# aniketntnu/WordDiffusion

Measured on AMD Instinct MI355X. Metric: denoised 64x256 word images/sec (1000-step DDPM), whole job, higher is better.
Workload: dtype bf16x3; 1 GPU; BASELINE configs[1]: batch 64 per GPU of 64x256 crops = [64,4,8,32] latents, 1000-step DDPM (999 executed steps), base unet.py UNetModel (320 ch, mult (1,1), 4 heads, 339 writers), random-init synthetic weights; variant=base, batch_per_gpu=64, noise_steps=1000, executed_steps_per_image=999, precision=split-bf16 MFMA x3, fp32 accumulate (<=1e-4 of the fp32 reference), output_finite=True

## Files before the change

worddiffusion_amd/csrc/wd_gemm.hip:

```cpp
#include <stdlib.h>

#include "wd_common.h"
#include "wd_gemm_epi.h"
#include "wd_gemm_priv.h"


namespace {

constexpr int BK = 32;

__device__ __forceinline__ int lds_off(int row, int ch) { return row * 64 + ((ch ^ ((row >> 2) & 3)) << 4); }
__device__ __forceinline__ int lds_off16(int row, int ch) { return row * 64 + ((ch ^ ((0 - (row >> 2)) & 3)) << 4); }


template <int BM, int BN, int TN, int NT>
__device__ __forceinline__ void wd_epilogue_lds(const wd_gemm_args& a, const f32x16 (&acc)[TN], char* smem, const int m0,
                                                const int n0, const int wm, const int wn, const int wcols, const int kh,
                                                const int nkh, const int tid, const int sidx = 0) {
    constexpr int LDE = BN + 4;
    float* ep = reinterpret_cast<float*>(smem);
    const int lane = tid & 63;
    const int frow = lane & 31, fhalf = lane >> 5;
    asm volatile("s_waitcnt vmcnt(0)" ::: "memory");
    __syncthreads();
// ... 2113 lines not shown
    if (a.rowvec && a.rowvec_ld <= 0) return WD_EINVAL;
    if (a.resid && a.resid_ld <= 0) return WD_EINVAL;
    {
        const int nout = a.act == WD_ACT_GEGLU ? a.n / 2 : a.n;
        if ((a.out_f32 && a.out_ld < nout) || (a.out_hi && a.out_pl_ld < nout) || (a.resid && a.resid_ld < nout) ||
            (a.rowvec && a.rowvec_ld < nout))
            return WD_EINVAL;
        for (int s = 0; s < a.nsrc; ++s)
            if (!(s == 0 && a.a32) && a.src[s].ld < a.src[s].c) return WD_EINVAL;
    }

    if (a.w_layout == 3) {
        bool ok = a.src[0].ntaps <= 9 && (a.nsrc == 1 || (a.src[1].gather == nullptr && a.src[1].ntaps == 1));
        for (int s = 0; s < a.nsrc; ++s) ok = ok && (a.src[s].c % 64 == 0);
        if (!ok) return WD_EINVAL;
        const wd_src& q0 = a.src[0];
        const bool same3 = q0.ntaps == 9 && q0.gather && a.slab_rows > 0 && q0.hw_src == a.hw_out && a.hw_out % a.slab_rows == 0;
        const bool down3 = a.tile == 64080 && q0.ntaps == 9 && q0.gather && a.slab_rows > 0 && q0.hw_src == 4 * a.hw_out;
        if (!same3 && !down3) a.slab_rows = 0;
        a.tickets = nullptr;
        if (a.tile == 64080) {
            if (!wd_gemmq_applies(a)) return WD_EINVAL;
            if (a.gn_gamma && (40 % a.gn_cpg || 80 % a.gn_cpg)) return WD_EINVAL;
            r.a = a, r.kernel = K_GEMMQ;
            return WD_OK;
        }
        const int nk64 = a.ktot / 64;
        if (a.ksplit == 0) a.ksplit = a.ws ? wd_auto_ksplit(a.tile, a.m, a.n, nk64, a.ws_floats) : 1;
        if (a.ksplit > 1 && (nk64 < a.ksplit || (long)a.ksplit * a.m * a.n > a.ws_floats)) a.ksplit = 1;
        if (a.gn_gamma && a.ksplit <= 1) return WD_EINVAL;
        {
            static const bool slab_env = getenv("WDIFF_GEMMW_SLAB") ? atoi(getenv("WDIFF_GEMMW_SLAB")) != 0 : WD_GEMMW_SLAB_DEFAULT;
            const bool want = (a.dbg & WD_GEMMW_SLAB_OFF) ? false : (a.dbg & WD_GEMMW_SLAB_ON) ? true : slab_env;
            const bool fits = a.tile == 64320 && a.npass == 3 && a.ksplit <= 1 && a.w_ngroups <= 1 && !a.a32 && !a.ln_gamma && same3 &&
                              64 % a.slab_rows == 0 && a.hw_out % 64 == 0 && a.m % a.hw_out == 0 && q0.c % 64 == 0 &&
                              (a.nsrc == 1 || (a.src[1].gather == nullptr && a.src[1].ntaps == 1));
            a.dbg &= ~(WD_GEMMW_SLAB_OFF | WD_GEMMW_SLAB_ON);
            if (want && fits) a.dbg |= WD_GEMMW_SLAB_BIT;
        }
        r.a = a, r.kernel = K_GEMMW;
        return WD_OK;
    }
#ifndef WDIFF_EXPERIMENTAL
    if (a.w_layout == 1) return WD_EINVAL;
#else
    if (a.w_layout == 1) {
        if (a.src[0].ntaps > 9 || a.slab_rows <= 0) return WD_EINVAL;
        if (a.nsrc == 2 && (a.src[1].gather || a.src[1].ntaps != 1)) return WD_EINVAL;
        if (a.tile == 0) a.tile = (a.act == WD_ACT_GEGLU || a.n % 160) ? 128064 : 128160;
        if (a.act == WD_ACT_GEGLU && a.n % (a.tile % 1000)) return WD_EINVAL;
        if (a.slab_rows > 192) return WD_EINVAL;
        if (a.tile != 128064 && a.tile != 128128 && a.tile != 128160) return WD_EINVAL;
        r.a = a, r.kernel = K_SLAB;
        return WD_OK;
    }
#endif
    bool conv3 = false;
    if (a.w_layout == 2) {
        const wd_src& q0 = a.src[0];
        static const int conv3_mode = getenv("WDIFF_CONV3") ? atoi(getenv("WDIFF_CONV3")) : 0;
#ifdef WDIFF_EXPERIMENTAL
        const bool conv3_env = conv3_mode != 0 || (a.dbg & 0x1000);
#else
        const bool conv3_env = false;
        (void)conv3_mode;
#endif
        const bool same3 = q0.ntaps == 9 && q0.gather && a.slab_rows > 0 && q0.hw_src == a.hw_out && a.hw_out % a.slab_rows == 0;
        conv3 = conv3_env && same3 && q0.c % 64 == 0 && a.act != WD_ACT_GEGLU && (a.tile == 0 || a.tile == 128160) &&
                (a.nsrc == 1 || (!a.src[1].gather && a.src[1].ntaps == 1 && a.src[1].c % 64 == 0));
        if (conv3) a.tile = 128160;
// ... 150 lines not shown
```

worddiffusion_amd/csrc/wd_gemm_priv.h:

```cpp
#pragma once
#include "wd_common.h"

int wd_gemmw_launch(const wd_gemm_args& a, hipStream_t st);
constexpr bool WD_GEMMW_SLAB_DEFAULT = true;
constexpr int WD_GEMMW_SLAB_OFF = 0x8000, WD_GEMMW_SLAB_ON = 0x10000, WD_GEMMW_SLAB_BIT = WD_GEMMW_SLAB_ON;
int wd_gemm_launch_reduce(const wd_gemm_args& a, hipStream_t st, int bm);
bool wd_gemmq_applies(const wd_gemm_args& a);
int wd_gemmq_launch(const wd_gemm_args& a, hipStream_t st);
```

worddiffusion_amd/csrc/wd_gemmw.hip:

```cpp
#include "wd_gemm_epi.h"
#include "wd_gemm_priv.h"

namespace {

constexpr int WNT = 512;

typedef __attribute__((ext_vector_type(4))) unsigned w_u32x4;

__device__ __forceinline__ int w_lds_off(int row, int ch) { return row * 128 + ((ch ^ ((row >> 1) & 7)) << 4); }

template <int NPASS, int RH, bool A32, bool SLAB = false>
__global__ void __launch_bounds__(WNT, 1) wd_gemmw_kernel(const wd_gemm_args a, const int nbn, const int nbm) {
#if defined(__HIP_DEVICE_COMPILE__)
    static_assert(!SLAB || (NPASS == 3 && RH == 1 && !A32), "the slab form is the split-bf16 64 x 320 kernel over operand planes");
    constexpr int NPL = (NPASS == 1) ? 1 : 2;
    constexpr int BM = 64 * RH, BN = 320 / RH;
    constexpr int A_PL = BM * 128;
    constexpr int STAGE = NPL * A_PL;
    constexpr uint32_t WD_OOB = 0x80000000u;

    extern __shared__ __attribute__((aligned(16))) char smem[];
    const int Wm = SLAB ? a.slab_rows : 1, wsh = __builtin_ctz(Wm);
    const int TR = 64 >> wsh, NR = TR + 2, SW = Wm + 2;
    const int CPL = NR * SW * 128, CHB = 2 * CPL;
    int* s_tab = reinterpret_cast<int*>(smem + 2 * STAGE);

    const int ntile = nbn * nbm;
    const int nwg = ntile * a.ksplit;
    int wg;
    {
        const int bid = blockIdx.x;
        const int q = nwg >> 3, r = nwg & 7, xcd = bid & 7, loc = bid >> 3;
        wg = (xcd < r ? xcd * (q + 1) : r * (q + 1) + (xcd - r) * q) + loc;
    }
    const int sidx = wg % a.ksplit;
    wg /= a.ksplit;
    const int bn_i = wg % nbn, bm_i = wg / nbn;
    const int m0 = bm_i * BM, n0 = bn_i * BN;

    const int tid = threadIdx.x;
    const int lane = tid & 63;
    const int wave = __builtin_amdgcn_readfirstlane(tid >> 6);
    const int kh = wave >> 2;
    const int rh = RH == 2 ? (wave >> 1) & 1 : 0;
    const int cg = RH == 2 ? wave & 1 : wave & 3;
    const int l15 = lane & 15, lq = lane >> 4;

    if constexpr (!SLAB) {
        const int nt0 = a.src[0].ntaps;
        const int32_t* g0 = a.src[0].gather;
        const int hw_src0 = a.src[0].hw_src;
        const int Wimg = a.slab_rows;
        for (int idx = tid; idx < nt0 * BM; idx += WNT) {
            const int t = idx / BM, row = idx - t * BM;
            const int m = m0 + row;
            int v = -1;
            if (m < a.m) {
                if (g0 && Wimg > 0) {
                    const int b = m / a.hw_out, p = m - b * a.hw_out;
                    const int y = p / Wimg, x = p - y * Wimg;
                    const int ky = t / 3, dy = ky - 1, dx = t - ky * 3 - 1;
                    const int sy = y + dy, sx = x + dx;
                    if (sy >= 0 && sy * Wimg < a.hw_out && sx >= 0 && sx < Wimg) v = b * hw_src0 + sy * Wimg + sx;
                } else if (g0) {
                    const int b = m / a.hw_out, p = m - b * a.hw_out;
                    const int g = g0[t * a.hw_out + p];
                    if (g >= 0) v = b * hw_src0 + g;
                } else {
                    v = m;
                }
            }
            s_tab[idx] = v;
        }
    }
    float* s_aff = reinterpret_cast<float*>(s_tab + 9 * BM);
    if constexpr (A32) {
        const int c0 = a.src[0].c;
        const int b = m0 / a.hw_out;
        const int ngp = c0 / a.a32_pcpg, ratio = a.a32_cpg / a.a32_pcpg;
        for (int c = tid; c < c0; c += WNT) {
            const int g = c / a.a32_cpg;
            double su = 0.0, sq = 0.0;
            for (int k = 0; k < ratio; ++k)
                for (int ck = 0; ck < a.a32_nchunk; ++ck) {
                    const double* pp = a.a32_part + (((long)b * a.a32_nchunk + ck) * ngp + g * ratio + k) * 2;
                    su += pp[0];
                    sq += pp[1];
                }
            const double n = (double)a.src[0].hw_src * a.a32_cpg;
            const double mu = su / n;
            double var = sq / n - mu * mu;
            if (var < 0.0) var = 0.0;
            const float rstd = (float)(1.0 / sqrt(var + (double)a.a32_eps));
            const float sc = rstd * a.a32_gamma[c];
            s_aff[2 * c] = sc;
            s_aff[2 * c + 1] = a.a32_beta[c] - (float)mu * sc;
        }
    }
    __syncthreads();
    unsigned long long skipmask = 0;
    if (!SLAB && RH == 1 && a.src[0].gather) {
        for (int t = 0; t < a.src[0].ntaps; ++t) {
            const unsigned long long oob = __ballot(s_tab[t * BM + lane] < 0);
#pragma unroll
            for (int i = 0; i < 4; ++i)
                if (((oob >> (16 * i)) & 0xFFFFull) == 0xFFFFull) skipmask |= 1ull << (4 * t + i);
        }
    }

    auto make_srd = [](const wd_bf16* p) {
        return __builtin_amdgcn_make_buffer_rsrc(const_cast<wd_bf16*>(p), 0, 0x7FFFFFF0, 0x00020000);
    };
    const int nct = a.n >> 4;
    const long wgrp = a.w_ngroups > 1 ? (long)((m0 % a.hw_out) / (a.hw_out / a.w_ngroups)) * a.w_group_stride : 0;
    const __amdgpu_buffer_rsrc_t srd_w_hi = make_srd(a.w_hi + wgrp), srd_w_lo = make_srd((a.w_lo ? a.w_lo : a.w_hi) + wgrp);
    const uint32_t b_voff = (uint32_t)(((n0 >> 4) + 5 * cg) * 1024 + lane * 16);
    const uint32_t kstep_bytes = (uint32_t)nct * 1024u;

    const int arow = tid >> 3, ach = tid & 7;
    const int a_dst = w_lds_off(arow, ach);

    const int nk_all = a.ktot / 64;
    const int cpt0 = a.src[0].c >> 6, n0st = a.src[0].ntaps * cpt0;
    const int k_begin = __builtin_amdgcn_readfirstlane((int)((long)nk_all * sidx / a.ksplit));
    const int k_end = __builtin_amdgcn_readfirstlane((int)((long)nk_all * (sidx + 1) / a.ksplit));
    const int nk = SLAB ? 0 : k_end - k_begin;
    int s = 0, tap = 0, kc = 0, left;
    int cur_ld = a.src[0].ld, cur_cpt = cpt0;
    if (k_begin < n0st) {
        tap = __builtin_amdgcn_readfirstlane(k_begin / cpt0);
        kc = k_begin - tap * cpt0;
// ... 153 lines not shown
                        acc[i][t] = __builtin_amdgcn_mfma_f32_16x16x32_bf16(xa[i][0], fb[t][NPL - 1], acc[i][t], 0, 0, 0);
                    }
                    acc[i][t] = __builtin_amdgcn_mfma_f32_16x16x32_bf16(xa[i][0], fb[t][0], acc[i][t], 0, 0, 0);
                }
            }
        }
    };
    const uint32_t cpt0_inv = (65536u + (uint32_t)cpt0 - 1u) / (uint32_t)cpt0;
    auto skip_of = [&](const int kit) {
        if constexpr (RH != 1) return 0;
        const int ka = k_begin + kit;
        const int tp = (int)(((uint32_t)ka * cpt0_inv) >> 16);
        int sk = (ka < n0st && ka < 1024) ? (int)((skipmask >> (4 * tp)) & 15ull) : 0;
        if (kit >= nk) sk = 15;
        return __builtin_amdgcn_readfirstlane(sk);
    };

    if constexpr (SLAB) {
        const wd_src& q0 = a.src[0];
        const int H = a.hw_out >> wsh;
        const int bsm = m0 / a.hw_out;
        const int y0 = (m0 - bsm * a.hw_out) >> wsh;
        const int ntok = NR * Wm;
        const int cpt1 = a.nsrc > 1 ? a.src[1].c >> 6 : 0, nch = cpt0 + cpt1;
        const int nst = 9 * cpt0 + cpt1;
        int skm0 = 0, skm2 = 0;
        int ub[4];
#pragma unroll
        for (int i = 0; i < 4; ++i) {
            if (y0 + ((16 * i + 15) >> wsh) < 1) skm0 |= 1 << i;
            if (y0 + ((16 * i) >> wsh) + 1 >= H) skm2 |= 1 << i;
            ub[i] = ((16 * i) >> wsh) * SW + ((16 * i) & (Wm - 1));
        }
        const uint32_t frow_bytes = (uint32_t)(q0.ld * 2), frow1_bytes = (uint32_t)(a.src[1].ld * 2);
        int fdst = -1;
        auto slab_piece = [&](const int t, const int chunk, const bool live) -> uint32_t {
            int ln;
            asm volatile("v_mbcnt_lo_u32_b32 %0, -1, 0\n\tv_mbcnt_hi_u32_b32 %0, -1, %0" : "=v"(ln));
            const int tq = wave * 8 + (ln >> 3) + 64 * t, fpc = ln & 7;
            if (chunk >= cpt0) {
                const bool piece = live && tq < 64;
                fdst = piece ? w_lds_off(tq, fpc) : -1;
                return piece ? (uint32_t)(m0 + tq) * frow1_bytes + (uint32_t)(fpc * 16) : WD_OOB;
            }
            const int fy = tq >> wsh, fx = tq & (Wm - 1);
            const int gy = y0 - 1 + fy;
            const bool piece = live && tq < ntok;
            fdst = piece ? w_lds_off(fy * SW + fx + 1, fpc) : -1;
            return (piece && gy >= 0 && gy < H) ? (uint32_t)(bsm * q0.hw_src + gy * Wm + fx) * frow_bytes + (uint32_t)(fpc * 16) : WD_OOB;
        };
        auto slab_load = [&](const int t, const int chunk, const bool live) {
            const uint32_t vo = slab_piece(t, chunk, live);
            if (chunk < cpt0) {
                ra[0][0] = __builtin_amdgcn_raw_buffer_load_b128(srd0_hi, vo, chunk * 128, 0);
                ra[0][1] = __builtin_amdgcn_raw_buffer_load_b128(srd0_lo, vo, chunk * 128, 0);
            } else {
                ra[0][0] = __builtin_amdgcn_raw_buffer_load_b128(srd1_hi, vo, (chunk - cpt0) * 128, 0);
                ra[0][1] = __builtin_amdgcn_raw_buffer_load_b128(srd1_lo, vo, (chunk - cpt0) * 128, 0);
            }
        };
        auto slab_store = [&](char* buf, const int t, const int chunk, const bool live) {
            slab_piece(t, chunk, live);
            if (fdst >= 0) {
                *reinterpret_cast<w_u32x4*>(buf + fdst) = ra[0][0];
                *reinterpret_cast<w_u32x4*>(buf + CPL + fdst) = ra[0][1];
            }
        };
        for (int i = tid; i < 2 * 2 * NR * 2 * 8; i += WNT) {
            const int pc = i & 7, side = (i >> 3) & 1;
            int rest = i >> 4;
            const int ry = rest % NR;
            rest /= NR;
            const int pl = rest & 1, bf = rest >> 1;
            *reinterpret_cast<w_u32x4*>(smem + bf * CHB + pl * CPL + w_lds_off(ry * SW + (side ? SW - 1 : 0), pc)) = w_u32x4{0u, 0u, 0u, 0u};
        }
        kb = 0;
        load_b(xb, true);
        {
            w_u32x4 v[3][2];
#pragma unroll
            for (int t = 0; t < 3; ++t) {
                slab_load(t, 0, true);
                v[t][0] = ra[0][0], v[t][1] = ra[0][1];
            }
#pragma unroll
            for (int t = 0; t < 3; ++t) {
                ra[0][0] = v[t][0], ra[0][1] = v[t][1];
                slab_store(smem, t, 0, true);
            }
        }
        int st = 0, sc = 0;
        int pft = 0, pfc = -1;
        auto mem_phase = [&](const int kit, bf16x8 (&bnext)[5][NPL]) {
            const bool conv = sc < cpt0;
            if (pfc >= 0) slab_store(smem + (pfc & 1) * CHB, pft, pfc, true);
            int tn = st + 1, cn = sc;
            if (tn == (conv ? 9 : 1)) tn = 0, cn = sc + 1;
            kb = cn < cpt0 ? tn * cpt0 + cn : n0st + cn - cpt0;
            load_b(bnext, kit + 1 < nst);
            const bool two = !conv || (st == 8 && sc == cpt0 - 1);
            const int fc = two ? sc + 2 : sc + 1, ft = two ? 0 : st;
            const bool freal = fc < nch && 64 * ft < (fc < cpt0 ? ntok : 64);
            pfc = freal ? fc : -1, pft = ft;
            if (freal) slab_load(ft, fc, true);
            const int ky = (st * 11) >> 5;
            const int shift = ky * SW + (st - 3 * ky);
            const char* cb = smem + (sc & 1) * CHB;
            int ln;
            asm volatile("v_mbcnt_lo_u32_b32 %0, -1, 0\n\tv_mbcnt_hi_u32_b32 %0, -1, %0" : "=v"(ln));
            const int f15 = ln & 15, ch = kh * 4 + (ln >> 4);
            const int frow = conv ? shift + (f15 >> wsh) * SW + (f15 & (Wm - 1)) : f15;
#pragma unroll
            for (int i = 0; i < 4; ++i) {
                const int ao = w_lds_off((conv ? ub[i] : 16 * i) + frow, ch);
#pragma unroll
                for (int p = 0; p < NPL; ++p) xa[i][p] = *reinterpret_cast<const bf16x8*>(cb + p * CPL + ao);
// ... 137 lines not shown
    const int nct = n >> 4;
    const int l = (int)(i & 63);
    const long blk = i >> 6;
    const int ct = (int)(blk % nct);
    const long ks = blk / nct;
    const long src = (long)(ct * 16 + (l & 15)) * ktot + ks * 32 + (l >> 4) * 8;
    reinterpret_cast<uint4*>(out_hi)[i] = *reinterpret_cast<const uint4*>(hi + src);
    if (lo) reinterpret_cast<uint4*>(out_lo)[i] = *reinterpret_cast<const uint4*>(lo + src);
}

template <int NPASS, int RH, bool A32 = false>
int launchw(const wd_gemm_args& a, hipStream_t st) {
    constexpr int NPL = (NPASS == 1) ? 1 : 2;
    constexpr int BM = 64 * RH, BN = 320 / RH;
    constexpr int loop_smem = 2 * NPL * BM * 128 + 9 * BM * 4 + (A32 ? 2 * 1024 * 4 : 0);
    constexpr int red_smem = BM * (BN + 4) * 4 + WD_STAT_SCRATCH;
    constexpr int smem = loop_smem > red_smem ? loop_smem : red_smem;
    static bool attr_done = false;
    if (!attr_done) {
        if (hipFuncSetAttribute(reinterpret_cast<const void*>(&wd_gemmw_kernel<NPASS, RH, A32>), hipFuncAttributeMaxDynamicSharedMemorySize,
                                smem) != hipSuccess)
            return WD_ELAUNCH;
        attr_done = true;
    }
    const int nbn = a.n / BN, nbm = (a.m + BM - 1) / BM;
    {
        WdLaunchScope scope(WD_CLS_GEMM_WDIRECT, st, 2.0 * (double)a.m * (double)a.n * (double)a.ktot);
        hipLaunchKernelGGL((wd_gemmw_kernel<NPASS, RH, A32>), dim3(nbn * nbm * a.ksplit), dim3(WNT), smem, st, a, nbn, nbm);
    }
    if (a.ksplit > 1) return wd_gemm_launch_reduce(a, st, BM);
    return wd_check_launch();
}

int launchw_slab(const wd_gemm_args& a, hipStream_t st) {
    constexpr int red_smem = 64 * (320 + 4) * 4 + WD_STAT_SCRATCH;
    constexpr int max_loop = 2 * 2 * 198 * 128;
    constexpr int max_smem = max_loop > red_smem ? max_loop : red_smem;
    static_assert(max_smem <= 160 * 1024, "LDS budget");
    const int W = a.slab_rows;
    const int loop_smem = 2 * 2 * (64 / W + 2) * (W + 2) * 128;
    const int smem = loop_smem > red_smem ? loop_smem : red_smem;
    static bool attr_done = false;
    if (!attr_done) {
        if (hipFuncSetAttribute(reinterpret_cast<const void*>(&wd_gemmw_kernel<3, 1, false, true>), hipFuncAttributeMaxDynamicSharedMemorySize,
                                max_smem) != hipSuccess)
            return WD_ELAUNCH;
        attr_done = true;
    }
    const int nbn = a.n / 320, nbm = a.m / 64;
    {
        WdLaunchScope scope(WD_CLS_GEMM_WDIRECT, st, 2.0 * (double)a.m * (double)a.n * (double)a.ktot);
        hipLaunchKernelGGL((wd_gemmw_kernel<3, 1, false, true>), dim3(nbn * nbm), dim3(WNT), smem, st, a, nbn, nbm);
    }
    return wd_check_launch();
}

}

int wd_gemmw_launch(const wd_gemm_args& a, hipStream_t st) {
    if (a.dbg & WD_GEMMW_SLAB_BIT) return launchw_slab(a, st);
    if (a.a32) return launchw<3, 1, true>(a, st);
    if (a.tile == 128160) return a.npass == 3 ? launchw<3, 2>(a, st) : launchw<1, 2>(a, st);
    return a.npass == 3 ? launchw<3, 1>(a, st) : launchw<1, 1>(a, st);
}

extern "C" int wd_gemm_pack_w(const wd_bf16* hi, const wd_bf16* lo, int n, int ktot, wd_bf16* out_hi, wd_bf16* out_lo, void* stream) {
    if (!hi || !out_hi || (lo && !out_lo) || n <= 0 || ktot <= 0 || n % 16 || ktot % 32) return WD_EINVAL;
    const long total = (long)n * ktot / 8;
    hipStream_t st = reinterpret_cast<hipStream_t>(stream);
    WdLaunchScope scope(WD_CLS_OTHER, st);
    hipLaunchKernelGGL(wd_pack_w_kernel, dim3((unsigned)((total + 255) / 256)), dim3(256), 0, st, hi, lo, n, ktot, out_hi, out_lo);
    return wd_check_launch();
}
```

worddiffusion_amd/engine.py:

```python
from __future__ import annotations

import collections
import ctypes as C
import math
import os
from typing import Dict, List, Optional, Tuple

import numpy as np
import torch

from . import _native as N
from .layers import (DownsampleParams, ResBlockParams, SpatialTransformerParams, UpsampleParams)


def conv_gather_table(h: int, w: int, mode: str) -> Tuple[np.ndarray, int, int]:
    if mode == "same":
        ho, wo = h, w
    elif mode == "down":
        ho, wo = (h + 2 - 3) // 2 + 1, (w + 2 - 3) // 2 + 1
    elif mode == "up":
        ho, wo = 2 * h, 2 * w
    elif mode == "down_rb":
        ho, wo = (h - 2) // 2 + 1, (w - 2) // 2 + 1
    else:
# ... 76 lines not shown
def slab_span(tab: Optional[np.ndarray], hw_out: int, hw_src: int, m: int, bm: int = 128) -> int:
    if tab is None:
        return bm
    period = int(np.lcm(bm, hw_out))
    mt = min(m, 2 * period)
    rows = np.arange(mt)
    b, p = rows // hw_out, rows % hw_out
    src = np.where(tab[:, p] >= 0, b[None, :] * hw_src + tab[:, p], -1)
    span = 0
    for r0 in range(0, mt, bm):
        blk = src[:, r0:r0 + bm]
        valid = blk[blk >= 0]
        if valid.size:
            span = max(span, int(valid.max() - valid.min() + 1))
    return span


_PARAM_GEN = [0]
_NATIVE_WRITES = [0]


def note_native_write():
    _NATIVE_WRITES[0] += 1

PLAN_CACHE_SIZE = int(os.environ.get("WDIFF_PLAN_CACHE", "4"))


def _bump_param_gen(*_a):
    _PARAM_GEN[0] += 1


torch.nn.modules.module.register_module_parameter_registration_hook(_bump_param_gen)

FILM_CHUNK_ROWS = int(os.environ.get("WDIFF_FILM_CHUNK_ROWS", "8192"))


class _Recipe:
    __slots__ = ("name", "planes", "rows", "cols", "shape", "pieces")

    def __init__(self, name, planes, rows=0, cols=0, shape=None):
        self.name, self.planes, self.rows, self.cols, self.shape, self.pieces = name, planes, rows, cols, shape, []

    @staticmethod
    def _nct(w):
        return w.shape[0], w.shape[1], (w.shape[2] * w.shape[3] if w.dim() == 4 else 1)

    def fwd(self, w, row_off=0, col_off=0, g=0):
        n, c, t = self._nct(w)
        assert row_off + n <= self.rows and col_off + t * c <= self.cols, self.name
        self.pieces.append((0, w, None, n, c, t, row_off, col_off, 0, g))
        return self

    def bwd(self, w, col_off=0, npad=None):
        n, c, t = self._nct(w)
        npad = n if npad is None else npad
        assert c <= self.rows and col_off + t * npad <= self.cols, self.name
        self.pieces.append((1, w, None, n, c, t, 0, col_off, npad, 0))
        return self

    def vec(self, p, p2=None, off=0, g=0):
        self.pieces.append((2, p, p2, p.numel(), 1, 1, 0, off, 0, g))
        return self

    def host(self) -> torch.Tensor:
        first = self.pieces[0][1]
        out = torch.zeros((self.rows, self.cols) if self.planes else (int(torch.tensor(self.shape).prod()),),
# ... 128 lines not shown
        raise ValueError(f"writer_keep must be a bool / uint8 tensor [{B}], False or None, got {k.dtype} {tuple(k.shape)}")
    return (k != 0).to(torch.uint8)


def _ptr(t: Optional[torch.Tensor], byte_off: int = 0):
    return None if t is None else t.data_ptr() + byte_off


class UNetEngine:

    fold_proj = False

    def __init__(self, model, variant: str):
        self.model = model
        self.variant = variant
        self.lib = N.lib()
        self.npass = 3
        self._sig = None
        self._ps, self._ps_gen = None, -1
        self._pack = None
        self._w: Dict[str, torch.Tensor] = {}
        self._w3: Dict[str, torch.Tensor] = {}
        self._w3_meta: Dict[str, tuple] = {}
        self._wf: Dict[str, torch.Tensor] = {}
        self.use_wdirect = os.environ.get("WDIFF_GEMM_WDIRECT", "1") != "0"
        self.gemmw_slab = {None: None, "0": False}.get(os.environ.get("WDIFF_GEMMW_SLAB"), True)
        self.use_up_phases = os.environ.get("WDIFF_UPSAMPLE_PHASES", "1") != "0"
        self._derived: Dict[str, tuple] = {}
        self.use_smallmap = os.environ.get("WDIFF_GEMM_SMALLMAP", "1") != "0"
        self.fuse_ff = os.environ.get("WDIFF_FUSE_FF", "1") != "0"
        self.fuse_proj = os.environ.get("WDIFF_FUSE_PROJ", "1") != "0"
        self.fuse_ln = os.environ.get("WDIFF_FUSE_LN", "1") != "0"
        self.fuse_gn_in = int(os.environ.get("WDIFF_FUSE_GN_IN", "1"))
        self.use_slab = os.environ.get("WDIFF_SLAB", "0") != "0"
        self.fuse_stats = os.environ.get("WDIFF_FUSE_STATS", "1") != "0"
        self.fuse_xattn = os.environ.get("WDIFF_FUSE_XATTN", "1") != "0"
        self.use_conv3 = os.environ.get("WDIFF_CONV3", "0") != "0"
        if (self.use_slab or self.use_conv3) and not self.lib.wd_gemm_experimental():
            raise N.NativeError("WDIFF_SLAB / WDIFF_CONV3 need a library built with WDIFF_EXPERIMENTAL=1 "
                                "(python -m worddiffusion_amd.build --force)")
        self.fuse_xattn_pair = os.environ.get("WDIFF_FUSE_XATTN_PAIR", "1") != "0"
        self.fuse_st = os.environ.get("WDIFF_FUSE_ST", "1") != "0"
        self.fold_proj = os.environ.get("WDIFF_FOLD_PROJ", "1") != "0"
        self.fuse_out = os.environ.get("WDIFF_FUSE_OUT", "1") != "0"
        self.fuse_in = os.environ.get("WDIFF_FUSE_IN", "1") != "0"
        self.pack_kv = os.environ.get("WDIFF_PACK_KV", "1") != "0"
        self.fuse_gn2 = os.environ.get("WDIFF_FUSE_GN2", "1") != "0"
        self.fuse_gn = os.environ.get("WDIFF_FUSE_GN", "1") != "0"
        self.fuse_split = os.environ.get("WDIFF_FUSE_SPLIT", "1") != "0"
        self._plans: Dict[tuple, Plan] = {}
        self._tabs: Dict[tuple, torch.Tensor] = {}
        self._tab_np: Dict[int, np.ndarray] = {}
        self._same_w: Dict[int, int] = {}
        self._down_w: Dict[int, int] = {}
        self._ws = None
        self.device = None

    def set_precision(self, mode: str):
        npass = {"bf16x3": 3, "fp32": 3, "bf16": 1}[mode]
        if npass != self.npass:
            self.npass = npass
            self._plans.clear()

    def _recipes(self) -> "RecipeBook":
        m = self.model
        R = RecipeBook()
# ... 246 lines not shown
        s.lo = planes[1].data_ptr() + 2 * col_off
        s.gather = _ptr(gather)
        s.ld, s.c, s.ntaps, s.hw_src = ld, c, ntaps, hw_src
        return s

    def _gemm(self, ops, what, srcs, wname, m, hw_out, bias=None, rowvec=None, rowvec_ld=0, resid=None,
              resid_ld=0, resid_rows=None, act=N.ACT_NONE, out_f32=None, out_ld=0, out_pl=None, n=None, tile=0,
              w_row_off=0, want_stats=False, a32=None, ln=None, w_groups=None):
        a = N.WdGemmArgs()
        for i, s in enumerate(srcs):
            a.src[i] = s
        a.nsrc = len(srcs)
        a.npass = self.npass
        wp = self._w[wname]
        ktot = wp.shape[2]
        assert ktot == sum(s.ntaps * s.c for s in srcs), (what, ktot, [(s.ntaps, s.c) for s in srcs])
        nrows = wp.shape[1] if n is None else n
        a.w_hi = wp[0].data_ptr() + 2 * w_row_off * ktot
        a.w_lo = wp[1].data_ptr() + 2 * w_row_off * ktot
        a.m, a.n, a.ktot, a.hw_out = m, nrows, ktot, hw_out
        a.bias = _ptr(bias)
        a.rowvec, a.rowvec_ld = rowvec, rowvec_ld
        a.resid, a.resid_ld, a.resid_rows = resid, resid_ld, resid_rows
        a.act = act
        a.out_f32, a.out_ld = _ptr(out_f32), out_ld
        if out_pl is not None:
            a.out_hi, a.out_lo, a.out_pl_ld = out_pl[0].data_ptr(), out_pl[1].data_ptr(), out_pl.shape[2]
        if a32 is not None:
            self._set_a32(a, *a32)
        if w_groups is not None:
            a.w_ngroups, a.w_group_stride = w_groups
        a.tile = tile
        if self._ws is None:
            self._ws = torch.empty(128 * 128 * 160 * 8, dtype=torch.float32, device=self.device)
        a.ksplit, a.ws, a.ws_floats = 0, self._ws.data_ptr(), self._ws.numel()
        self._give_tickets(a, m, nrows)
        span = 0
        if self.use_slab and w_row_off == 0 and (len(srcs) == 1 or (srcs[1].ntaps == 1 and not srcs[1].gather)):
            tabnp = getattr(srcs[0], "_tab_np", None)
            span = slab_span(tabnp, hw_out, srcs[0].hw_src, m)
            if span > 192 or ((m + 127) // 128) * max(1, nrows // 160) < 96:
                span = 0
        s0 = srcs[0]
        frag = not span and not self.use_conv3 and w_row_off == 0 and n is None and act == N.ACT_NONE and tile == 0
        width = (getattr(s0, "_down_w", 0) or getattr(s0, "_same_w", 0)) if s0.ntaps == 9 else 0
        wdirect = (frag and self.use_wdirect and wdirect_fills_chip(m, nrows) and
                   self._legal(a, w_layout=3, tile=64320, slab_rows=getattr(s0, "_same_w", 0) if s0.ntaps == 9 else 0))
        smallmap = (frag and not wdirect and self.use_smallmap and hw_out == 64 and 128 <= (m // 64) * (nrows // 80) <= 512 and
                    self._legal(a, w_layout=3, tile=64080, slab_rows=width))
        assert (a32 is None and w_groups is None) or wdirect, what
        if wdirect or smallmap:
            wf = self._wfrag(wname)
            a.w_hi, a.w_lo = wf[0].data_ptr(), wf[1].data_ptr()
            if wdirect and self.gemmw_slab is not None:
                a.dbg |= 0x10000 if self.gemmw_slab else 0x8000
        elif span:
            meta = (srcs[0].ntaps, srcs[0].c, srcs[1].c if len(srcs) > 1 else 0)
            if wname not in self._w3:
                self._w3[wname] = slab_order(wp, *meta)
                self._w3_meta[wname] = meta
            assert self._w3_meta[wname] == meta, wname
            w3 = self._w3[wname]
            a.w_hi, a.w_lo = w3[0].data_ptr(), w3[1].data_ptr()
            a.w_layout, a.slab_rows = 1, span
        else:
            same_w = getattr(srcs[0], "_same_w", 0)
            if (same_w and srcs[0].ntaps == 9 and srcs[0].c % 64 == 0 and act == N.ACT_NONE and tile == 0 and
                    (len(srcs) == 1 or (srcs[1].ntaps == 1 and not srcs[1].gather and srcs[1].c % 64 == 0))):
                a.w_layout, a.slab_rows = 2, same_w
        a._ln_pl = None
        if ln is not None and self.fuse_ln and not self.use_slab:
            pl = torch.zeros((2, m, nrows), dtype=torch.bfloat16, device=self.device)
            if self._legal(a, out_hi=pl[0].data_ptr(), out_lo=pl[1].data_ptr(), out_pl_ld=nrows, ln_gamma=self._w[ln + ".g"].data_ptr(),
                           ln_beta=self._w[ln + ".b"].data_ptr(), ln_eps=1e-5):
                self._cur_plan.keep.append(pl)
                a._ln_pl = pl
        stats = None
        if want_stats and self.fuse_stats and nrows % 32 == 0 and (hw_out % 128 == 0 or hw_out == 64) and not span:
            cpg = nrows // 32
            r = self._resolved(a, stat_part=a.ws, stat_cpg=cpg)
            if r is not None:
                nchunk = max(1, hw_out // (r.tile // 1000))
                part = torch.zeros((m // hw_out, nchunk, 32, 2), dtype=torch.float64, device=self.device)
                self._cur_plan.keep.append(part)
                a.stat_part, a.stat_cpg = part.data_ptr(), cpg
                stats = (part, nchunk, cpg)
        a._stats = stats
        self._cur_plan.keep.append(a)
        ops.append((self.lib.wd_gemm, (C.byref(a),), what))
        return a

    def _resolved(self, a, **fields) -> Optional[N.WdGemmArgs]:
        b = N.WdGemmArgs.from_buffer_copy(a)
        for k, v in fields.items():
            setattr(b, k, v)
        out = N.WdGemmArgs()
        return out if self.lib.wd_gemm_check(C.byref(b), C.byref(out)) == N.WD_OK else None

    def _legal(self, a, apply=True, **fields) -> bool:
        if self._resolved(a, **fields) is None:
            return False
        if apply:
            for k, v in fields.items():
                setattr(a, k, v)
        return True

    def _set_a32(self, a, x32: "Act", gname, eps, silu):
        part, nchunk, pc = x32.stats
        a.a32, a.a32_ld, a.a32_part = x32.t.data_ptr(), x32.c, part.data_ptr()
        a.a32_nchunk, a.a32_pcpg, a.a32_cpg = nchunk, pc, x32.c // 32
        a.a32_gamma, a.a32_beta = self._w[gname + ".g"].data_ptr(), self._w[gname + ".b"].data_ptr()
        a.a32_eps, a.a32_silu = float(eps), int(silu)

    def _wdirect_ok(self, srcs, m, n, hw_out, a32=None, **fields) -> bool:
        a = N.WdGemmArgs()
        for i, s in enumerate(srcs):
            a.src[i] = s
        a.nsrc, a.npass, a.m, a.n, a.ktot, a.hw_out = len(srcs), self.npass, m, n, sum(s.ntaps * s.c for s in srcs), hw_out
        a.w_layout, a.tile = 3, 64320
        a.w_hi = a.w_lo = a.out_f32 = 16
        a.out_ld = n
        if a32 is not None:
            self._set_a32(a, *a32)
        return self._legal(a, apply=False, **fields)

    def _give_tickets(self, a, m, n):
        ntick = ((m + 63) // 64) * ((n + 63) // 64)
        if ntick > 2048:
            return
        P = self._cur_plan
        tk = getattr(P, "_tickets", None)
        if tk is None or P._ticket_off + ntick > tk.numel():
            tk = torch.zeros(1 << 16, dtype=torch.int32, device=self.device)
            P.keep.append(tk)
            P._tickets, P._ticket_off = tk, 0
        a.tickets, a.ntickets = tk.data_ptr() + 4 * P._ticket_off, ntick
        P._ticket_off += ntick

    def _gn(self, P, ops, what, srcs: List[Act], gname, eps, silu, want_raw=False, dropout=None):
        B = self._B
        h, w = srcs[0].h, srcs[0].w
        hw = h * w
        ctot = sum(s.c for s in srcs)
        cpg = ctot // 32
        has_perm = any(s.perm is not None for s in srcs)
        if has_perm and not (len(srcs) == 2 and srcs[1].perm is None and self.fuse_gn2 and not any(s.c % cpg for s in srcs)):
            raise NotImplementedError(f"{what}: a phase-major map (Upsample) is read by the two-source GroupNorm of a decoder block only")
        if any(s.c % cpg for s in srcs):
            cat = self._f32(P, B * hw, ctot)
            coff = 0
            for s in srcs:
                ops.append((self.lib.wd_copy2d, (cat.data_ptr() + 4 * coff, 4 * ctot, s.t.data_ptr(), 4 * s.c, 4 * s.c,
                                                 B * hw), what + ":concat"))
                coff += s.c
            srcs = [Act(cat, ctot, h, w)]
        pl = self._planes(P, B * hw, ctot)
        raw = self._planes(P, B * hw, ctot) if want_raw else None
# ... 19 lines not shown
        rhi, rlo = self._hilo(raw)
        if len(todo) == 2 and self.fuse_gn2:
            (sa, pa, na, pca, ca), (sb, pb, nb_, pcb, cb) = todo
            ops.append((self.lib.wd_gn_apply2,
                        (sa.t.data_ptr(), sa.c, sa.c, pa.data_ptr(), na, pca, ca, sb.t.data_ptr(), sb.c, sb.c, pb.data_ptr(), nb_, pcb, cb,
                         B, hw, cpg, gam.data_ptr(), bet.data_ptr(), eps, int(silu), hi, lo, ctot, rhi, rlo,
                         sa.perm.data_ptr() if sa.perm is not None else None),
                        what + ":apply"))
        elif dropout is not None:
            assert not has_perm and len(srcs) == 1, what
            (s, part, nchunk, pc, c0), = todo
            ops.append((self.lib.wd_gn_apply_dropout,
                        (s.t.data_ptr(), s.c, B, hw, s.c, cpg, part.data_ptr(), nchunk, pc, gam.data_ptr(), bet.data_ptr(), eps,
                         int(silu), hi, lo, ctot, c0, rhi, rlo, C.byref(dropout)), what + ":apply+dropout"))
        else:
            assert not has_perm, what
            for s, part, nchunk, pc, c0 in todo:
                ops.append((self.lib.wd_gn_apply,
                            (s.t.data_ptr(), s.c, B, hw, s.c, cpg, part.data_ptr(), nchunk, pc, gam.data_ptr(), bet.data_ptr(), eps,
                             int(silu), hi, lo, ctot, c0, rhi, rlo), what + ":apply"))
        return pl, raw

    def _gn_stats(self, P, ops, what, s: Act):
        if s.stats is None:
            B, hw = self._B, s.h * s.w
            nchunk = self.lib.wd_gn_nchunk(hw)
            pc = s.c // 32
            part = torch.empty((B, nchunk, 32, 2), dtype=torch.float64, device=self.device)
            P.keep.append(part)
            ops.append((self.lib.wd_gn_stats, (s.t.data_ptr(), s.c, B, hw, s.c, pc, part.data_ptr()), what + ":stats"))
            s.stats = (part, nchunk, pc)
        return s.stats

    def _gn_in_consumer(self, P, ops, what, srcs: List[Act], want_raw, M, hw, ncols, taps=1, gather=None) -> bool:
        if not (self.fuse_gn_in and self.use_wdirect and len(srcs) == 1 and not want_raw and not self.use_conv3):
            return False
        if taps > 1 and self.fuse_gn_in < 2:
            return False
        if not wdirect_fills_chip(M, ncols):
            return False
        s = srcs[0]
        self._gn_stats(P, ops, what, s)
        return self._wdirect_ok([self._src32(s, taps, gather, hw)], M, ncols, hw, a32=(s, what, 0.0, False))

    def _src32(self, x: Act, ntaps=1, gather=None, hw_src=0) -> N.WdSrc:
        s = N.WdSrc()
        s._tab_np = self._tab_np.get(gather.data_ptr()) if gather is not None else None
        s._same_w = self._same_w.get(gather.data_ptr(), 0) if gather is not None else 0
        s.hi, s.lo, s.gather = None, None, _ptr(gather)
        s.ld, s.c, s.ntaps, s.hw_src = x.c, x.c, ntaps, hw_src
        return s

    def _gn_in_combine(self, s: Act, raw, gam, bet, eps, silu, cpg, pl, coff) -> bool:
        pr = s.prod
        if pr is None or not isinstance(pr, N.WdGemmArgs) or not self.fuse_gn or raw is not None or self.use_conv3:
            return False
        if pr.out_f32 != s.t.data_ptr() or pr.out_hi or pr.gn_gamma or pr.n != s.c:
            return False
        hi, lo = self._hilo(pl, 2 * coff)
        return self._legal(pr, gn_gamma=gam.data_ptr() + 4 * coff, gn_beta=bet.data_ptr() + 4 * coff, gn_eps=float(eps),
                           gn_silu=int(silu), gn_cpg=cpg, out_hi=hi, out_lo=lo, out_pl_ld=pl.shape[2])

    def _ln(self, P, ops, what, x: torch.Tensor, rows, c, name):
        pl = self._planes(P, rows, c)
        ops.append((self.lib.wd_layernorm,
                    (x.data_ptr(), c, rows, c, self._w[name + ".g"].data_ptr(), self._w[name + ".b"].data_ptr(), 1e-5,
                     *self._hilo(pl), c), what))
        return pl

    def _resblock(self, P, name, mod: ResBlockParams, srcs: List[Act]) -> Act:
        ops = P.step
        B = self._B
        h, w = srcs[0].h, srcs[0].w
        hw, M = h * w, B * h * w
        cin, cout = mod.cin, mod.cout
        assert cin == sum(s.c for s in srcs)
        tab, _, _ = self._table(h, w, "same")
        need_raw = cin != cout
        h1 = self._f32(P, M, cout)
        if self._gn_in_consumer(P, ops, name + ".gn1", srcs, need_raw, M, hw, cout, taps=9, gather=tab):
            s1, in1 = self._src32(srcs[0], 9, tab, hw), (srcs[0], name + ".gn1", 1e-5, True)
            raw = None
        else:
            a1, raw = self._gn(P, ops, name + ".gn1", srcs, name + ".gn1", 1e-5, True, want_raw=need_raw)
            s1, in1 = self._src(a1, cin, 9, tab, hw), None
        g1 = self._gemm(ops, name + ".conv1", [s1], name + ".c1.w", M, hw,
                        bias=self._w[name + ".c1.b"], rowvec=self._film.data_ptr() + 4 * self.film_off[name],
                        rowvec_ld=self.film_total, out_f32=h1, out_ld=cout, want_stats=True, a32=in1)
        h1a = Act(h1, cout, h, w, g1._stats, prod=g1)
        if self._gn_in_consumer(P, ops, name + ".gn2", [h1a], False, M, hw, cout, taps=9, gather=tab):
            s2, in2 = self._src32(h1a, 9, tab, hw), (h1a, name + ".gn2", 1e-5, True)
        else:
            a2, _ = self._gn(P, ops, name + ".gn2", [h1a], name + ".gn2", 1e-5, True)
            s2, in2 = self._src(a2, cout, 9, tab, hw), None
        out = self._f32(P, M, cout)
        if need_raw:
            g2 = self._gemm(ops, name + ".conv2+skip", [s2, self._src(raw, cin)],
                            name + ".c2.w", M, hw, bias=self._w[name + ".c2.b"], out_f32=out, out_ld=cout,
                            want_stats=True, a32=in2)
        else:
            g2 = self._gemm(ops, name + ".conv2", [s2], name + ".c2.w", M, hw,
                            bias=self._w[name + ".c2.b"], resid=srcs[0].t.data_ptr(), resid_ld=cout, out_f32=out,
                            out_ld=cout, want_stats=True, a32=in2)
        return Act(out, cout, h, w, g2._stats, prod=g2)

    def _up_phases_ok(self, mod) -> bool:
        return (getattr(self, "use_up_phases", False) and self.use_wdirect and self.fuse_gn2 and self.npass == 3 and not self.use_slab and
                not self.use_conv3)

    def _resample(self, P, name, mod, x: Act, mode: str, tile: int = 0) -> Act:
        ops = P.step
        B = self._B
        assert x.perm is None, name
        tab, ho, wo = self._table(x.h, x.w, mode)
        pl = self._planes(P, B * x.h * x.w, x.c)
        pr = x.prod
        if (pr is not None and self.fuse_split and not pr.out_hi and pr.out_f32 == x.t.data_ptr() and
                (pr.n if isinstance(pr, N.WdGemmArgs) else pr.c) == x.c):
            pr.out_hi, pr.out_lo = self._hilo(pl)
            pr.out_pl_ld = x.c
        else:
            ops.append((self.lib.wd_split, (x.t.data_ptr(), x.c, B * x.h * x.w, x.c, 0, *self._hilo(pl), x.c), name + ":split"))
        out = self._f32(P, B * ho * wo, mod.cout)
# ... 739 lines not shown
```

Baseline: 37.39 images/s.

## Fuse GroupNorm+SiLU input into slab-form 3x3 conv GEMM kernel

Extends the slab-tiled split-bf16 3x3 conv kernel to take fp32 activations and apply the GroupNorm affine and SiLU while staging into LDS, splitting into hi/lo bf16 planes on the fly. The per-channel affine table is built in shared memory after the first slab loads are issued. The engine now routes 3x3 GN-consumer convolutions to this path by default when the slab form applies, which removes the separate GN kernel and its bf16 plane write and read. In exchange the kernel reads twice the bytes per element in fp32, does extra ALU work in the staging path and uses more LDS.

After: 37.68 images/s, median of 6. No clear change (+0.8%).

```diff
diff --git a/worddiffusion_amd/csrc/wd_gemm.hip b/worddiffusion_amd/csrc/wd_gemm.hip
--- a/worddiffusion_amd/csrc/wd_gemm.hip
+++ b/worddiffusion_amd/csrc/wd_gemm.hip
@@ -2169,10 +2169,10 @@
         {
             static const bool slab_env = getenv("WDIFF_GEMMW_SLAB") ? atoi(getenv("WDIFF_GEMMW_SLAB")) != 0 : WD_GEMMW_SLAB_DEFAULT;
             const bool want = (a.dbg & WD_GEMMW_SLAB_OFF) ? false : (a.dbg & WD_GEMMW_SLAB_ON) ? true : slab_env;
-            const bool fits = a.tile == 64320 && a.npass == 3 && a.ksplit <= 1 && a.w_ngroups <= 1 && !a.a32 && !a.ln_gamma && same3 &&
+            const bool fits = a.tile == 64320 && a.npass == 3 && a.ksplit <= 1 && a.w_ngroups <= 1 && (!a.a32 || (a.dbg & WD_GEMMW_SLAB_A32)) && !a.ln_gamma && same3 &&
                               64 % a.slab_rows == 0 && a.hw_out % 64 == 0 && a.m % a.hw_out == 0 && q0.c % 64 == 0 &&
                               (a.nsrc == 1 || (a.src[1].gather == nullptr && a.src[1].ntaps == 1));
-            a.dbg &= ~(WD_GEMMW_SLAB_OFF | WD_GEMMW_SLAB_ON);
+            a.dbg &= ~(WD_GEMMW_SLAB_OFF | WD_GEMMW_SLAB_ON | WD_GEMMW_SLAB_A32);
             if (want && fits) a.dbg |= WD_GEMMW_SLAB_BIT;
         }
         r.a = a, r.kernel = K_GEMMW;
diff --git a/worddiffusion_amd/csrc/wd_gemm_priv.h b/worddiffusion_amd/csrc/wd_gemm_priv.h
--- a/worddiffusion_amd/csrc/wd_gemm_priv.h
+++ b/worddiffusion_amd/csrc/wd_gemm_priv.h
@@ -4,6 +4,7 @@
 int wd_gemmw_launch(const wd_gemm_args& a, hipStream_t st);
 constexpr bool WD_GEMMW_SLAB_DEFAULT = true;
 constexpr int WD_GEMMW_SLAB_OFF = 0x8000, WD_GEMMW_SLAB_ON = 0x10000, WD_GEMMW_SLAB_BIT = WD_GEMMW_SLAB_ON;
+constexpr int WD_GEMMW_SLAB_A32 = 0x20000;
 int wd_gemm_launch_reduce(const wd_gemm_args& a, hipStream_t st, int bm);
 bool wd_gemmq_applies(const wd_gemm_args& a);
 int wd_gemmq_launch(const wd_gemm_args& a, hipStream_t st);
diff --git a/worddiffusion_amd/csrc/wd_gemmw.hip b/worddiffusion_amd/csrc/wd_gemmw.hip
--- a/worddiffusion_amd/csrc/wd_gemmw.hip
+++ b/worddiffusion_amd/csrc/wd_gemmw.hip
@@ -8,11 +8,34 @@
 typedef __attribute__((ext_vector_type(4))) unsigned w_u32x4;
 
 __device__ __forceinline__ int w_lds_off(int row, int ch) { return row * 128 + ((ch ^ ((row >> 1) & 7)) << 4); }
+
+__device__ __forceinline__ void w_aff_table(const wd_gemm_args& a, float* s_aff, const int b, const int tid) {
+    const int c0 = a.src[0].c;
+    const int ngp = c0 / a.a32_pcpg, ratio = a.a32_cpg / a.a32_pcpg;
+    for (int c = tid; c < c0; c += WNT) {
+        const int g = c / a.a32_cpg;
+        double su = 0.0, sq = 0.0;
+        for (int k = 0; k < ratio; ++k)
+            for (int ck = 0; ck < a.a32_nchunk; ++ck) {
+                const double* pp = a.a32_part + (((long)b * a.a32_nchunk + ck) * ngp + g * ratio + k) * 2;
+                su += pp[0];
+                sq += pp[1];
+            }
+        const double n = (double)a.src[0].hw_src * a.a32_cpg;
+        const double mu = su / n;
+        double var = sq / n - mu * mu;
+        if (var < 0.0) var = 0.0;
+        const float rstd = (float)(1.0 / sqrt(var + (double)a.a32_eps));
+        const float sc = rstd * a.a32_gamma[c];
+        s_aff[2 * c] = sc;
+        s_aff[2 * c + 1] = a.a32_beta[c] - (float)mu * sc;
+    }
+}
 
 template <int NPASS, int RH, bool A32, bool SLAB = false>
 __global__ void __launch_bounds__(WNT, 1) wd_gemmw_kernel(const wd_gemm_args a, const int nbn, const int nbm) {
 #if defined(__HIP_DEVICE_COMPILE__)
-    static_assert(!SLAB || (NPASS == 3 && RH == 1 && !A32), "the slab form is the split-bf16 64 x 320 kernel over operand planes");
+    static_assert(!SLAB || (NPASS == 3 && RH == 1), "the slab form is the split-bf16 64 x 320 kernel");
     constexpr int NPL = (NPASS == 1) ? 1 : 2;
     constexpr int BM = 64 * RH, BN = 320 / RH;
     constexpr int A_PL = BM * 128;
@@ -73,30 +96,8 @@
             s_tab[idx] = v;
         }
     }
-    float* s_aff = reinterpret_cast<float*>(s_tab + 9 * BM);
-    if constexpr (A32) {
-        const int c0 = a.src[0].c;
-        const int b = m0 / a.hw_out;
-        const int ngp = c0 / a.a32_pcpg, ratio = a.a32_cpg / a.a32_pcpg;
-        for (int c = tid; c < c0; c += WNT) {
-            const int g = c / a.a32_cpg;
-            double su = 0.0, sq = 0.0;
-            for (int k = 0; k < ratio; ++k)
-                for (int ck = 0; ck < a.a32_nchunk; ++ck) {
-                    const double* pp = a.a32_part + (((long)b * a.a32_nchunk + ck) * ngp + g * ratio + k) * 2;
-                    su += pp[0];
-                    sq += pp[1];
-                }
-            const double n = (double)a.src[0].hw_src * a.a32_cpg;
-            const double mu = su / n;
-            double var = sq / n - mu * mu;
-            if (var < 0.0) var = 0.0;
-            const float rstd = (float)(1.0 / sqrt(var + (double)a.a32_eps));
-            const float sc = rstd * a.a32_gamma[c];
-            s_aff[2 * c] = sc;
-            s_aff[2 * c + 1] = a.a32_beta[c] - (float)mu * sc;
-        }
-    }
+    float* s_aff = (A32 && SLAB) ? reinterpret_cast<float*>(smem + 2 * CHB) : reinterpret_cast<float*>(s_tab + 9 * BM);
+    if constexpr (A32 && !SLAB) w_aff_table(a, s_aff, m0 / a.hw_out, tid);
     __syncthreads();
     unsigned long long skipmask = 0;
     if (!SLAB && RH == 1 && a.src[0].gather) {
@@ -316,8 +317,13 @@
             if (y0 + ((16 * i) >> wsh) + 1 >= H) skm2 |= 1 << i;
             ub[i] = ((16 * i) >> wsh) * SW + ((16 * i) & (Wm - 1));
         }
+        if constexpr (A32) {
+            skm0 = __builtin_amdgcn_readfirstlane(skm0);
+            skm2 = __builtin_amdgcn_readfirstlane(skm2);
+        }
         const uint32_t frow_bytes = (uint32_t)(q0.ld * 2), frow1_bytes = (uint32_t)(a.src[1].ld * 2);
         int fdst = -1;
+        int fch = -1;
         auto slab_piece = [&](const int t, const int chunk, const bool live) -> uint32_t {
             int ln;
             asm volatile("v_mbcnt_lo_u32_b32 %0, -1, 0\n\tv_mbcnt_hi_u32_b32 %0, -1, %0" : "=v"(ln));
@@ -325,19 +331,30 @@
             if (chunk >= cpt0) {
                 const bool piece = live && tq < 64;
                 fdst = piece ? w_lds_off(tq, fpc) : -1;
+                if constexpr (A32) fch = -1;
                 return piece ? (uint32_t)(m0 + tq) * frow1_bytes + (uint32_t)(fpc * 16) : WD_OOB;
             }
             const int fy = tq >> wsh, fx = tq & (Wm - 1);
             const int gy = y0 - 1 + fy;
             const bool piece = live && tq < ntok;
             fdst = piece ? w_lds_off(fy * SW + fx + 1, fpc) : -1;
+            if constexpr (A32) {
+                const bool inside = piece && gy >= 0 && gy < H;
+                fch = inside ? chunk * 64 + fpc * 8 : -1;
+                return inside ? (uint32_t)(bsm * q0.hw_src + gy * Wm + fx) * (uint32_t)(a.a32_ld * 4) + (uint32_t)(fpc * 32) : WD_OOB;
+            }
             return (piece && gy >= 0 && gy < H) ? (uint32_t)(bsm * q0.hw_src + gy * Wm + fx) * frow_bytes + (uint32_t)(fpc * 16) : WD_OOB;
         };
         auto slab_load = [&](const int t, const int chunk, const bool live) {
             const uint32_t vo = slab_piece(t, chunk, live);
             if (chunk < cpt0) {
-                ra[0][0] = __builtin_amdgcn_raw_buffer_load_b128(srd0_hi, vo, chunk * 128, 0);
-                ra[0][1] = __builtin_amdgcn_raw_buffer_load_b128(srd0_lo, vo, chunk * 128, 0);
+                if constexpr (A32) {
+                    ra[0][0] = __builtin_amdgcn_raw_buffer_load_b128(srd0_hi, vo, chunk * 256, 0);
+                    ra[0][1] = __builtin_amdgcn_raw_buffer_load_b128(srd0_hi, vo + 16, chunk * 256, 0);
+                } else {
+                    ra[0][0] = __builtin_amdgcn_raw_buffer_load_b128(srd0_hi, vo, chunk * 128, 0);
+                    ra[0][1] = __builtin_amdgcn_raw_buffer_load_b128(srd0_lo, vo, chunk * 128, 0);
+                }
             } else {
                 ra[0][0] = __builtin_amdgcn_raw_buffer_load_b128(srd1_hi, vo, (chunk - cpt0) * 128, 0);
                 ra[0][1] = __builtin_amdgcn_raw_buffer_load_b128(srd1_lo, vo, (chunk - cpt0) * 128, 0);
@@ -345,6 +362,27 @@
         };
         auto slab_store = [&](char* buf, const int t, const int chunk, const bool live) {
             slab_piece(t, chunk, live);
+            if constexpr (A32) {
+                if (fdst >= 0 && chunk < cpt0) {
+                    const float4* tab = reinterpret_cast<const float4*>(s_aff + 2 * (fch >= 0 ? fch : 0));
+                    const float4 t0 = tab[0], t1 = tab[1], t2 = tab[2], t3 = tab[3];
+                    const float4 x0 = __builtin_bit_cast(float4, ra[0][0]), x1 = __builtin_bit_cast(float4, ra[0][1]);
+                    float4 y0, y1;
+                    y0.x = x0.x * t0.x + t0.y; y0.y = x0.y * t0.z + t0.w; y0.z = x0.z * t1.x + t1.y; y0.w = x0.w * t1.z + t1.w;
+                    y1.x = x1.x * t2.x + t2.y; y1.y = x1.y * t2.z + t2.w; y1.z = x1.z * t3.x + t3.y; y1.w = x1.w * t3.z + t3.w;
+                    if (a.a32_silu != 0) {
+                        y0.x = wd_silu(y0.x); y0.y = wd_silu(y0.y); y0.z = wd_silu(y0.z); y0.w = wd_silu(y0.w);
+                        y1.x = wd_silu(y1.x); y1.y = wd_silu(y1.y); y1.z = wd_silu(y1.z); y1.w = wd_silu(y1.w);
+                    }
+                    if (fch < 0) y0 = y1 = make_float4(0.f, 0.f, 0.f, 0.f);
+                    uint2 h0, l0, h1, l1;
+                    wd_split4(y0, h0, l0);
+                    wd_split4(y1, h1, l1);
+                    *reinterpret_cast<w_u32x4*>(buf + fdst) = w_u32x4{h0.x, h0.y, h1.x, h1.y};
+                    *reinterpret_cast<w_u32x4*>(buf + CPL + fdst) = w_u32x4{l0.x, l0.y, l1.x, l1.y};
+                    return;
+                }
+            }
             if (fdst >= 0) {
                 *reinterpret_cast<w_u32x4*>(buf + fdst) = ra[0][0];
                 *reinterpret_cast<w_u32x4*>(buf + CPL + fdst) = ra[0][1];
@@ -366,6 +404,10 @@
             for (int t = 0; t < 3; ++t) {
                 slab_load(t, 0, true);
                 v[t][0] = ra[0][0], v[t][1] = ra[0][1];
+            }
+            if constexpr (A32) {
+                w_aff_table(a, s_aff, bsm, tid);
+                __syncthreads();
             }
 #pragma unroll
             for (int t = 0; t < 3; ++t) {
@@ -569,17 +611,18 @@
     return wd_check_launch();
 }
 
+template <bool A32>
 int launchw_slab(const wd_gemm_args& a, hipStream_t st) {
     constexpr int red_smem = 64 * (320 + 4) * 4 + WD_STAT_SCRATCH;
-    constexpr int max_loop = 2 * 2 * 198 * 128;
+    constexpr int max_loop = 2 * 2 * 198 * 128 + (A32 ? 2 * 1024 * 4 : 0);
     constexpr int max_smem = max_loop > red_smem ? max_loop : red_smem;
     static_assert(max_smem <= 160 * 1024, "LDS budget");
     const int W = a.slab_rows;
-    const int loop_smem = 2 * 2 * (64 / W + 2) * (W + 2) * 128;
+    const int loop_smem = 2 * 2 * (64 / W + 2) * (W + 2) * 128 + (A32 ? 2 * a.src[0].c * 4 : 0);
     const int smem = loop_smem > red_smem ? loop_smem : red_smem;
     static bool attr_done = false;
     if (!attr_done) {
-        if (hipFuncSetAttribute(reinterpret_cast<const void*>(&wd_gemmw_kernel<3, 1, false, true>), hipFuncAttributeMaxDynamicSharedMemorySize,
+        if (hipFuncSetAttribute(reinterpret_cast<const void*>(&wd_gemmw_kernel<3, 1, A32, true>), hipFuncAttributeMaxDynamicSharedMemorySize,
                                 max_smem) != hipSuccess)
             return WD_ELAUNCH;
         attr_done = true;
@@ -587,7 +630,7 @@
     const int nbn = a.n / 320, nbm = a.m / 64;
     {
         WdLaunchScope scope(WD_CLS_GEMM_WDIRECT, st, 2.0 * (double)a.m * (double)a.n * (double)a.ktot);
-        hipLaunchKernelGGL((wd_gemmw_kernel<3, 1, false, true>), dim3(nbn * nbm), dim3(WNT), smem, st, a, nbn, nbm);
+        hipLaunchKernelGGL((wd_gemmw_kernel<3, 1, A32, true>), dim3(nbn * nbm), dim3(WNT), smem, st, a, nbn, nbm);
     }
     return wd_check_launch();
 }
@@ -595,7 +638,7 @@
 }
 
 int wd_gemmw_launch(const wd_gemm_args& a, hipStream_t st) {
-    if (a.dbg & WD_GEMMW_SLAB_BIT) return launchw_slab(a, st);
+    if (a.dbg & WD_GEMMW_SLAB_BIT) return a.a32 ? launchw_slab<true>(a, st) : launchw_slab<false>(a, st);
     if (a.a32) return launchw<3, 1, true>(a, st);
     if (a.tile == 128160) return a.npass == 3 ? launchw<3, 2>(a, st) : launchw<1, 2>(a, st);
     return a.npass == 3 ? launchw<3, 1>(a, st) : launchw<1, 1>(a, st);
diff --git a/worddiffusion_amd/engine.py b/worddiffusion_amd/engine.py
--- a/worddiffusion_amd/engine.py
+++ b/worddiffusion_amd/engine.py
@@ -132,6 +132,8 @@
 
 torch.nn.modules.module.register_module_parameter_registration_hook(_bump_param_gen)
 
+WS_FLOATS = 128 * 128 * 160 * 8
+GN_IN_SLAB_DEFAULT = "1"
 FILM_CHUNK_ROWS = int(os.environ.get("WDIFF_FILM_CHUNK_ROWS", "8192"))
 
 
@@ -326,6 +328,7 @@
         self.fuse_proj = os.environ.get("WDIFF_FUSE_PROJ", "1") != "0"
         self.fuse_ln = os.environ.get("WDIFF_FUSE_LN", "1") != "0"
         self.fuse_gn_in = int(os.environ.get("WDIFF_FUSE_GN_IN", "1"))
+        self.gn_in_slab = os.environ.get("WDIFF_GN_IN_SLAB", GN_IN_SLAB_DEFAULT) != "0"
         self.use_slab = os.environ.get("WDIFF_SLAB", "0") != "0"
         self.fuse_stats = os.environ.get("WDIFF_FUSE_STATS", "1") != "0"
         self.fuse_xattn = os.environ.get("WDIFF_FUSE_XATTN", "1") != "0"
@@ -638,7 +641,7 @@
             a.w_ngroups, a.w_group_stride = w_groups
         a.tile = tile
         if self._ws is None:
-            self._ws = torch.empty(128 * 128 * 160 * 8, dtype=torch.float32, device=self.device)
+            self._ws = torch.empty(WS_FLOATS, dtype=torch.float32, device=self.device)
         a.ksplit, a.ws, a.ws_floats = 0, self._ws.data_ptr(), self._ws.numel()
         self._give_tickets(a, m, nrows)
         span = 0
@@ -658,8 +661,9 @@
         if wdirect or smallmap:
             wf = self._wfrag(wname)
             a.w_hi, a.w_lo = wf[0].data_ptr(), wf[1].data_ptr()
-            if wdirect and self.gemmw_slab is not None:
-                a.dbg |= 0x10000 if self.gemmw_slab else 0x8000
+            if wdirect:
+                a.dbg |= self._slab_dbg(a32 is not None and s0.ntaps == 9)
+                assert a32 is None or s0.ntaps != 9 or self.fuse_gn_in >= 2 or self._resolved(a).dbg & 0x10000, what
         elif span:
             meta = (srcs[0].ntaps, srcs[0].c, srcs[1].c if len(srcs) > 1 else 0)
             if wname not in self._w3:
@@ -711,14 +715,21 @@
                 setattr(a, k, v)
         return True
 
+    def _slab_dbg(self, a32_3x3: bool) -> int:
+        dbg = 0 if self.gemmw_slab is None else 0x10000 if self.gemmw_slab else 0x8000
+        return dbg | (0x20000 if a32_3x3 and self.gn_in_slab else 0)
+
     def _set_a32(self, a, x32: "Act", gname, eps, silu):
-        part, nchunk, pc = x32.stats
-        a.a32, a.a32_ld, a.a32_part = x32.t.data_ptr(), x32.c, part.data_ptr()
+        part, nchunk, pc = x32.stats if x32.stats is not None else (None, 1, x32.c // 32)
+        a.a32, a.a32_ld, a.a32_part = x32.t.data_ptr(), x32.c, part.data_ptr() if part is not None else 16
         a.a32_nchunk, a.a32_pcpg, a.a32_cpg = nchunk, pc, x32.c // 32
         a.a32_gamma, a.a32_beta = self._w[gname + ".g"].data_ptr(), self._w[gname + ".b"].data_ptr()
         a.a32_eps, a.a32_silu = float(eps), int(silu)
 
     def _wdirect_ok(self, srcs, m, n, hw_out, a32=None, **fields) -> bool:
+        return self._wdirect_resolved(srcs, m, n, hw_out, a32, **fields) is not None
+
+    def _wdirect_resolved(self, srcs, m, n, hw_out, a32=None, **fields) -> Optional[N.WdGemmArgs]:
         a = N.WdGemmArgs()
         for i, s in enumerate(srcs):
             a.src[i] = s
@@ -728,7 +739,7 @@
         a.out_ld = n
         if a32 is not None:
             self._set_a32(a, *a32)
-        return self._legal(a, apply=False, **fields)
+        return self._resolved(a, **fields)
 
     def _give_tickets(self, a, m, n):
         ntick = ((m + 63) // 64) * ((n + 63) // 64)
@@ -814,14 +825,20 @@
             s.stats = (part, nchunk, pc)
         return s.stats
 
-    def _gn_in_consumer(self, P, ops, what, srcs: List[Act], want_raw, M, hw, ncols, taps=1, gather=None) -> bool:
+    def _gn_in_consumer(self, P, ops, what, srcs: List[Act], want_raw, M, hw, ncols, taps=1, gather=None, more=()) -> bool:
         if not (self.fuse_gn_in and self.use_wdirect and len(srcs) == 1 and not want_raw and not self.use_conv3):
-            return False
-        if taps > 1 and self.fuse_gn_in < 2:
             return False
         if not wdirect_fills_chip(M, ncols):
             return False
         s = srcs[0]
+        if taps > 1 and self.fuse_gn_in < 2:
+            if not (self.gn_in_slab and self.gemmw_slab is not False):
+                return False
+            r = self._wdirect_resolved([self._src32(s, taps, gather, hw), *more], M, ncols, hw, a32=(s, what, 0.0, False),
+                                       slab_rows=self._same_w.get(gather.data_ptr(), 0), dbg=self._slab_dbg(True), ws=16,
+                                       ws_floats=WS_FLOATS)
+            if r is None or not r.dbg & 0x10000:
+                return False
         self._gn_stats(P, ops, what, s)
         return self._wdirect_ok([self._src32(s, taps, gather, hw)], M, ncols, hw, a32=(s, what, 0.0, False))
 
@@ -870,7 +887,8 @@
                         bias=self._w[name + ".c1.b"], rowvec=self._film.data_ptr() + 4 * self.film_off[name],
                         rowvec_ld=self.film_total, out_f32=h1, out_ld=cout, want_stats=True, a32=in1)
         h1a = Act(h1, cout, h, w, g1._stats, prod=g1)
-        if self._gn_in_consumer(P, ops, name + ".gn2", [h1a], False, M, hw, cout, taps=9, gather=tab):
+        if self._gn_in_consumer(P, ops, name + ".gn2", [h1a], False, M, hw, cout, taps=9, gather=tab,
+                                more=[self._src(raw, cin)] if need_raw else []):
             s2, in2 = self._src32(h1a, 9, tab, hw), (h1a, name + ".gn2", 1e-5, True)
         else:
             a2, _ = self._gn(P, ops, name + ".gn2", [h1a], name + ".gn2", 1e-5, True)
```
